# DillionLowry/NeuralCodecs

Measured on AMD Instinct MI355X. Metric: audio-seconds/sec encode+decode (x real-time), DAC-44.1kHz B=32, higher is better.
Workload: dtype f32; 1 GPU; DAC 44.1kHz 8kbps encode+decode, batch=32 x 1 s clips per GPU (BASELINE configs[1]); clips_per_gpu=32, global_batch=32, collective=none

## Files before the change

include/nc_mi355x.h:

```cpp
#ifndef NC_MI355X_H
#define NC_MI355X_H

#include <stddef.h>
#include <stdint.h>

#ifdef __cplusplus
extern "C" {
#endif

#define NC_API __attribute__((visibility("default")))

typedef enum {
    NC_OK = 0,
    NC_EINVAL = 1,
    NC_ENOTFOUND = 2,
    NC_ESTATE = 3,
    NC_EDEVICE = 4,
    NC_ENOMEM = 5,
    NC_EUNSUPPORTED = 6
} nc_status;

typedef struct nc_codec nc_codec;

NC_API const char* nc_last_error(void);
// ... 212 lines not shown
    NC_KC_COUNT = 13
} nc_kernel_class;

typedef struct {
    int64_t launches;
    double ms;
    double flops;
    double bytes;
} nc_profile_entry;

NC_API nc_status nc_codec_profile_enable(nc_codec* h, int32_t on);
NC_API nc_status nc_codec_profile_reset(nc_codec* h);
NC_API nc_status nc_codec_profile_read(nc_codec* h, nc_profile_entry* out);

typedef struct {
    int32_t B, Cin, Cout, K, stride, pad, dil, out_pad;
    int64_t Tin;
    int32_t transposed;
    int32_t tanh_out;
} nc_conv_desc;

NC_API nc_status nc_op_conv1d(int device_index, const nc_conv_desc* d, const float* x, const float* weight, const float* bias,
                              const float* alpha_in, const float* alpha_out, const float* residual, float* y, int64_t* Tout);
NC_API nc_status nc_op_conv1d_bench(int device_index, const nc_conv_desc* d, int32_t fuse, int32_t iters, double* avg_ms);
NC_API nc_status nc_op_res_unit(int device_index, int32_t B, int32_t C, int64_t T, int32_t dil, const float* x, const float* w7,
                                const float* b7, const float* a1, const float* a2, const float* w1, const float* b1,
                                int32_t fused, float* y, int32_t iters, double* avg_ms);
NC_API nc_status nc_op_vq_argmin(int device_index, const float* z_e, int32_t B, int32_t D, int64_t T, const float* codebook,
                                 int32_t N, int64_t* idx, float* st);
NC_API nc_status nc_op_euclid_rvq(int device_index, const float* residual, int32_t B, int32_t D, int64_t T, const float* codebooks,
                                  int32_t n_q, int32_t N, int32_t form, int64_t* codes, float* residual_out);
NC_API nc_status nc_op_fold_weight_norm(const float* v, const float* g, int64_t d0, int64_t inner, float* w);
NC_API nc_status nc_op_dwconv1d(int device_index, int32_t B, int32_t C, int64_t T, int32_t K, int32_t pad, int32_t dil, const float* x,
                                const float* w, const float* bias, const float* alpha_in, const float* alpha_out, float* y);
NC_API nc_status nc_op_layer_norm(int device_index, int32_t B, int32_t C, int64_t T, const float* x, const float* gamma,
                                  const float* beta, float* y);
NC_API nc_status nc_op_local_attn(int device_index, int32_t B, int32_t C, int64_t T, int32_t W, const float* qkv, const float* inv_freq,
                                  float* y);
NC_API nc_status nc_op_avg_pool(int device_index, int64_t rows, int64_t T, int32_t s, const float* x, float* y);
NC_API nc_status nc_op_snac_unit(int device_index, int32_t B, int32_t C, int64_t T, int32_t dil, const float* x, const float* w7,
                                 const float* b7, const float* a1, const float* a2, const float* w1, const float* b1,
                                 const float* alpha_next, int32_t fused, float* y);

#ifdef __cplusplus
}
#endif
// ... 2 lines not shown
```

neuralcodecs_amd/_lib.py:

```python
from __future__ import annotations

import ctypes as C
import os
import sys

_HERE = os.path.dirname(os.path.abspath(__file__))
LIB_PATH = os.path.join(_HERE, "libnc_mi355x.so")

NC_OK, NC_EINVAL, NC_ENOTFOUND, NC_ESTATE, NC_EDEVICE, NC_ENOMEM, NC_EUNSUPPORTED = range(7)
NC_KC_NAMES = ("conv_k7", "conv_k1", "conv_down", "conv_up", "conv_misc", "rvq", "elem", "dwconv", "norm", "attn", "lstm", "stem", "head")


class NcError(RuntimeError):
    """Base of engine errors (the reference's NeuralCodecException, Core/Exceptions/NeuralCodecException.cs:10-73)."""


class NcDeviceError(NcError):
    pass


class NcDacConfig(C.Structure):
    _fields_ = [("sample_rate", C.c_int32), ("encoder_dim", C.c_int32), ("n_encoder_rates", C.c_int32),
                ("encoder_rates", C.c_int32 * 8), ("decoder_dim", C.c_int32), ("n_decoder_rates", C.c_int32),
                ("decoder_rates", C.c_int32 * 8), ("latent_dim", C.c_int32), ("n_codebooks", C.c_int32),
# ... 108 lines not shown
    ("nc_audio_deinterleave_dev", C.c_int, [C.c_int, _P, C.c_int64, C.c_int32, _P, _P]),
    ("nc_audio_resample_linear_dev", C.c_int, [C.c_int, _P, C.c_int32, C.c_int64, C.c_int32, C.c_int32, _P, _P]),
    ("nc_group_unique_id", C.c_int, [_P]),
    ("nc_group_create_rank", C.c_int, [C.c_int32, C.c_int32, _P, _P, C.POINTER(_P)]),
    ("nc_group_create_local", C.c_int, [C.c_int32, C.POINTER(_P), C.POINTER(_P)]),
    ("nc_group_create_local_ex", C.c_int, [C.c_int32, C.POINTER(_P), C.c_uint32, C.POINTER(_P)]),
    ("nc_group_destroy", C.c_int, [_P]),
    ("nc_group_info", C.c_int, [_P, C.POINTER(C.c_int32), C.POINTER(C.c_int32)]),
    ("nc_group_set_code_bits", C.c_int, [_P, C.c_int32]),
    ("nc_group_dac_encode_allgather_dev", C.c_int, [_P, _P, C.c_int32, C.c_int64, C.c_int32, C.c_int32, _P, _P, _P]),
    ("nc_group_snac_encode_allgather_dev", C.c_int, [_P, _P, C.c_int32, C.c_int64, _P]),
    ("nc_group_wait", C.c_int, [_P]),
    ("nc_group_dac_encode_allgather", C.c_int, [_P, _P, C.c_int32, C.c_int64, C.c_int32, C.c_int32, _P, _P]),
    ("nc_group_snac_encode_allgather", C.c_int, [_P, _P, C.c_int32, C.c_int64, _P]),
    ("nc_group_dac_encode_allgather_local_dev", C.c_int, [_P, C.POINTER(_P), C.POINTER(C.c_int32), C.c_int64, C.c_int32, C.c_int32, C.POINTER(_P),
                                                          C.POINTER(_P), C.POINTER(_P)]),
    ("nc_group_snac_encode_allgather_local_dev", C.c_int, [_P, C.POINTER(_P), C.POINTER(C.c_int32), C.c_int64, C.POINTER(_P)]),
    ("nc_group_encodec_encode_allgather_dev", C.c_int, [_P, _P, C.c_int32, C.c_int64, _P, _P]),
    ("nc_group_encodec_encode_allgather_local_dev", C.c_int, [_P, C.POINTER(_P), C.POINTER(C.c_int32), C.c_int64, C.POINTER(_P), C.POINTER(_P)]),
    ("nc_codec_profile_enable", C.c_int, [_P, C.c_int32]),
    ("nc_codec_profile_reset", C.c_int, [_P]),
    ("nc_codec_profile_read", C.c_int, [_P, C.POINTER(NcProfileEntry)]),
    ("nc_op_conv1d", C.c_int, [C.c_int, C.POINTER(NcConvDesc), _P, _P, _P, _P, _P, _P, _P, C.POINTER(C.c_int64)]),
    ("nc_op_conv1d_bench", C.c_int, [C.c_int, C.POINTER(NcConvDesc), C.c_int32, C.c_int32, C.POINTER(C.c_double)]),
    ("nc_op_res_unit", C.c_int, [C.c_int, C.c_int32, C.c_int32, C.c_int64, C.c_int32, _P, _P, _P, _P, _P, _P, _P, C.c_int32, _P,
                                 C.c_int32, C.POINTER(C.c_double)]),
    ("nc_op_vq_argmin", C.c_int, [C.c_int, _P, C.c_int32, C.c_int32, C.c_int64, _P, C.c_int32, _P, _P]),
    ("nc_op_euclid_rvq", C.c_int, [C.c_int, _P, C.c_int32, C.c_int32, C.c_int64, _P, C.c_int32, C.c_int32, C.c_int32, _P, _P]),
    ("nc_op_fold_weight_norm", C.c_int, [_P, _P, C.c_int64, C.c_int64, _P]),
    ("nc_op_dwconv1d", C.c_int, [C.c_int, C.c_int32, C.c_int32, C.c_int64, C.c_int32, C.c_int32, C.c_int32, _P, _P, _P, _P, _P, _P]),
    ("nc_op_layer_norm", C.c_int, [C.c_int, C.c_int32, C.c_int32, C.c_int64, _P, _P, _P, _P]),
    ("nc_op_local_attn", C.c_int, [C.c_int, C.c_int32, C.c_int32, C.c_int64, C.c_int32, _P, _P, _P]),
    ("nc_op_avg_pool", C.c_int, [C.c_int, C.c_int64, C.c_int64, C.c_int32, _P, _P]),
    ("nc_op_snac_unit", C.c_int, [C.c_int, C.c_int32, C.c_int32, C.c_int64, C.c_int32, _P, _P, _P, _P, _P, _P, _P, _P, C.c_int32, _P]),
]


def lib():
    global _lib
    if _lib is not None:
        return _lib
    path = os.environ.get("NC_MI355X_LIB") or LIB_PATH
    if not os.path.exists(path):
        raise NcError(f"{path} is missing: build it with `python -c 'import __graft_entry__ as g; g.build()'` "
                      "(make -C neuralcodecs_amd/csrc). There is no fallback implementation.")
    if "torch" not in sys.modules:
# ... 73 lines not shown
```

neuralcodecs_amd/csrc/nc_api.hip:

```cpp
#include <algorithm>
#include <cmath>
#include <cstdio>
#include <fstream>

#include "nc_model.h"

using namespace nc;


namespace {

template <class F>
nc_status guard(F&& f) {
    try {
        f();
        return NC_OK;
    } catch (const Error& e) {
        set_last_error(e.what());
        return e.code;
    } catch (const std::bad_alloc&) {
        set_last_error("host allocation failed");
        return NC_ENOMEM;
    } catch (const std::exception& e) {
        set_last_error(e.what());
// ... 671 lines not shown
    return guard([&] {
        if (!d || !x || !weight || !y) fail(NC_EINVAL, "null argument");
        if (d->B <= 0 || d->Cin <= 0 || d->Cout <= 0 || d->K <= 0 || d->stride <= 0 || d->Tin <= 0) fail(NC_EINVAL, "bad conv shape");
        op_set_device(device_index);
        ConvLayer L;
        L.build(weight, bias, d->Cin, d->Cout, d->K, d->stride, d->pad, d->dil, d->out_pad, d->transposed != 0);
        const int64_t Tout = L.out_len(d->Tin);
        if (Tout <= 0) fail(NC_EINVAL, "empty output");
        if (Tout_p) *Tout_p = Tout;
        DevBuf dx, dy, dai, dao, dr;
        const size_t nx = (size_t)d->B * d->Cin * d->Tin * 4, ny = (size_t)d->B * d->Cout * Tout * 4;
        dx.reserve(nx); dy.reserve(ny);
        NC_HIP(hipMemcpy(dx.p, x, nx, hipMemcpyHostToDevice));
        NC_HIP(hipMemset(dy.p, 0, ny));
        if (alpha_in) { dai.reserve(d->Cin * 4); NC_HIP(hipMemcpy(dai.p, alpha_in, d->Cin * 4, hipMemcpyHostToDevice)); }
        if (alpha_out) { dao.reserve(d->Cout * 4); NC_HIP(hipMemcpy(dao.p, alpha_out, d->Cout * 4, hipMemcpyHostToDevice)); }
        if (residual) { dr.reserve(ny); NC_HIP(hipMemcpy(dr.p, residual, ny, hipMemcpyHostToDevice)); }
        ConvIO io{};
        io.x = dx.as<float>(); io.x_bstride = (int64_t)d->Cin * d->Tin; io.x_cstride = d->Tin; io.x_len = (int32_t)d->Tin; io.Tin = d->Tin;
        io.alpha_in = alpha_in ? dai.as<float>() : nullptr;
        io.alpha_out = alpha_out ? dao.as<float>() : nullptr;
        io.res = residual ? dr.as<float>() : nullptr;
        io.y = dy.as<float>(); io.y_bstride = (int64_t)d->Cout * Tout; io.y_cstride = Tout;
        io.epi = d->tanh_out ? EPI_TANH : 0;
        launch_conv(L, io, d->B, nullptr, nullptr);
        NC_HIP(hipDeviceSynchronize());
        NC_HIP(hipMemcpy(y, dy.p, ny, hipMemcpyDeviceToHost));
        dx.release(); dy.release(); dai.release(); dao.release(); dr.release(); L.release_all();
    });
}

nc_status nc_op_conv1d_bench(int device_index, const nc_conv_desc* d, int32_t fuse, int32_t iters, double* avg_ms) {
    return guard([&] {
        if (!d || !avg_ms || iters <= 0) fail(NC_EINVAL, "null argument");
        if (d->B <= 0 || d->Cin <= 0 || d->Cout <= 0 || d->K <= 0 || d->stride <= 0 || d->Tin <= 0) fail(NC_EINVAL, "bad conv shape");
        op_set_device(device_index);
        uint64_t st = 0x9E3779B97F4A7C15ull;
        auto rnd = [&]() {
            st = st * 6364136223846793005ull + 1442695040888963407ull;
            return (float)((int64_t)(st >> 40) - (1 << 23)) * (1.0f / (1 << 23));
        };
        const size_t nw = (size_t)d->Cin * d->Cout * d->K;
        std::vector<float> w(nw), bias(d->Cout), al(std::max(d->Cin, d->Cout));
        const float sc = 1.0f / std::sqrt((float)d->Cin * (d->transposed ? 2 : d->K));
        for (auto& v : w) v = rnd() * sc;
        for (auto& v : bias) v = rnd() * 0.1f;
// ... 260 lines not shown
```

neuralcodecs_amd/csrc/nc_chunk.hip:

```cpp
#include <algorithm>

#include "nc_limits.h"
#include "nc_model.h"

namespace nc {

namespace {

int64_t ceil_div(int64_t a, int64_t b) { return (a + b - 1) / b; }
int64_t round_up(int64_t a, int64_t m) { return ceil_div(a, m) * m; }

void halo_from_layers(const int32_t* er, int ne, const int32_t* dr, int nd, int final_reach, int W, int vq_max, int64_t align, nc_halo* out) {
    if (ne <= 0 || ne > 8 || nd <= 0 || nd > 8) fail(NC_EINVAL, "encoder/decoder rate lists must hold 1..8 entries");
    int64_t l = final_reach, r = final_reach, hop = 1;
    if (W > 1) { l += W - 1; r += W - 1; }
    for (int i = ne - 1; i >= 0; --i) {
        const int64_t s = er[i], p = (s + 1) / 2;
        if (s <= 0) fail(NC_EINVAL, "encoder rate must be positive");
        l = l * s + p; r = r * s + (2 * s - 1 - p);
        l += 39; r += 39;
        hop *= s;
    }
    l += 3; r += 3;
    int64_t a = 3, b = 3, H = 1;
    if (W > 1) { a += W - 1; b += W - 1; }
    for (int i = 0; i < nd; ++i) {
        const int64_t s = dr[i], p = (s + 1) / 2;
        if (s <= 0) fail(NC_EINVAL, "decoder rate must be positive");
        a = a * s + p; b = b * s + (2 * s - 1 - p);
        a += 39; b += 39;
        H *= s;
    }
    a += 3; b += 3;
    out->align = align;
    out->enc_left = round_up(ceil_div(r, hop) + (vq_max - 1), align);
    out->enc_right = round_up(ceil_div(l, hop) + (vq_max - 1), align);
    out->dec_left = round_up(ceil_div(a, H), align);
    out->dec_right = round_up(ceil_div(b, H), align);
}

int64_t pitch16(int64_t L) { return L >= 256 ? ((L + 15) & ~(int64_t)15) : L; }

int64_t auto_chunk(const nc_halo& h, bool decode) {
    const int64_t hmax = decode ? std::max(h.dec_left, h.dec_right) : std::max(h.enc_left, h.enc_right);
    return round_up(std::max<int64_t>(1024, 16 * hmax), h.align);
}

bool oneshot_fits(const int32_t* er, int ne, int enc_dim, const int32_t* dr, int nd, int dec_dim, ChunkKind kind, int64_t frames) {
    const int bm = 512;
    if (kind == CK_ENCODE) {
        int64_t L = frames;
        for (int i = 0; i < ne; ++i) L *= er[i];
        if (L > ((int64_t)1 << 30)) return false;
        return conv_rows_fit32(bm, pitch16(L), L);
    }
    if (kind == CK_DECODE) {
        int64_t L = frames;
        for (int i = 0; i < nd; ++i) {
            const int64_t s = dr[i], Lo = L * s, P = pitch16(Lo);
            const int Co = dec_dim >> (i + 1);
            if (!conv_rows_fit32(bm, P, Lo) || !conv_subpixel_fits32(Co, P, (int64_t)Co * P, Lo)) return false;
            L = Lo;
        }
        return true;
// ... 326 lines not shown
```

neuralcodecs_amd/csrc/nc_conv.hip:

```cpp
#include <algorithm>
#include <cstdlib>
#include <mutex>
#include <set>

#include "nc_conv.h"
#include "nc_limits.h"

namespace nc {

typedef void (*conv_kernel_fn)(const ConvArgs);
conv_kernel_fn conv_kernel_table_k1(int, int);
int conv_kernel_cb_k1();
int conv_kernel_nx_k1();
conv_kernel_fn conv_kernel_table_k2(int, int);
int conv_kernel_cb_k2();
int conv_kernel_nx_k2();
conv_kernel_fn conv_kernel_table_k3(int, int);
int conv_kernel_cb_k3();
int conv_kernel_nx_k3();
conv_kernel_fn conv_kernel_table_k4(int, int);
int conv_kernel_cb_k4();
int conv_kernel_nx_k4();
conv_kernel_fn conv_kernel_table_k6(int, int);
int conv_kernel_cb_k6();
int conv_kernel_nx_k6();
conv_kernel_fn conv_kernel_table_k7(int, int);
int conv_kernel_cb_k7();
int conv_kernel_nx_k7();
conv_kernel_fn conv_kernel_table_k8(int, int);
int conv_kernel_cb_k8();
int conv_kernel_nx_k8();
conv_kernel_fn conv_kernel_table_k10(int, int);
int conv_kernel_cb_k10();
int conv_kernel_nx_k10();
conv_kernel_fn conv_kernel_table_k16(int, int);
int conv_kernel_cb_k16();
int conv_kernel_nx_k16();

#define NC_K_CASES(X) X(1) X(2) X(3) X(4) X(6) X(7) X(8) X(10) X(16)

conv_kernel_fn conv_kernel_table_fused_k7(int, int);
conv_kernel_fn conv_kernel_table_xv_k7(int);
conv_kernel_fn conv_kernel_table_xv_fused_k7(int);
conv_kernel_fn conv_kernel_table_xv_sub_k2(int);
conv_kernel_fn conv_kernel_table_xv_subg_k2(int);
conv_kernel_fn conv_kernel_table_sub_k2(int, int);
conv_kernel_fn conv_kernel_table_subg_k2(int, int);
conv_kernel_fn conv_kernel_table_dist_k16(int, int);
conv_kernel_fn conv_kernel_table_dist_sub_k2(int, int);
conv_kernel_fn conv_kernel_table_sub_narrow_k2(int);
conv_kernel_fn conv_kernel_table_fusedw_k7(int, int);
conv_kernel_fn conv_kernel_table_slim_k3(int, int);
conv_kernel_fn conv_kernel_table_slim_k7(int, int);
conv_kernel_fn conv_kernel_table_narrow_k2(int);
conv_kernel_fn conv_kernel_table_narrow_k3(int);
conv_kernel_fn conv_kernel_table_narrow_k7(int);
conv_kernel_fn conv_kernel_table_narrow_k16(int);
static conv_kernel_fn narrow_kernel(int K, int TM) {
    switch (K) {
        case 2: return conv_kernel_table_narrow_k2(TM);
        case 3: return conv_kernel_table_narrow_k3(TM);
        case 7: return conv_kernel_table_narrow_k7(TM);
        case 16: return conv_kernel_table_narrow_k16(TM);
    }
    return nullptr;
}
conv_kernel_fn conv_kernel_table_in2_k4(int, int);
conv_kernel_fn conv_kernel_table_in2_k8(int, int);
// ... 602 lines not shown
        if (io.epi & EPI_NOISE) fail(NC_ESTATE, "internal: noise epilogue on the multiply-shift sub-pixel form");
        a.sub_stride = L.sub_stride; a.sub_cout = L.Cout; a.sub_magic = magic_div(L.sub_stride, L.rows() + 256);
        if (!conv_subpixel_fits32(L.Cout, io.y_cstride, io.y_bstride, Tout))
            fail(NC_EUNSUPPORTED, "conv output of %lld samples per row exceeds the 32-bit offsets of the sub-pixel form", (long long)io.y_cstride);
    }
    a.Tout = (int32_t)Tout;
    if (!conv_rows_fit32(c.BM(), io.y_cstride, Tout))
        fail(NC_EUNSUPPORTED, "conv output rows of %lld samples exceed the 32-bit tile offsets", (long long)io.y_cstride);
    int sx;
    if (L.transposed) {
        sx = 1; a.stride = 1; a.dil = -1; a.pad = 0;
        a.n_cols = (int32_t)(io.Tin + L.Ktaps - 1);
        a.y_tstride = L.stride; a.y_toff = -L.pad;
        a.n_phase = L.n_phase;
    } else {
        sx = L.stride; a.stride = L.stride; a.dil = L.dil; a.pad = L.pad;
        a.n_cols = (int32_t)Tout;
        a.y_tstride = 1; a.y_toff = 0;
        a.n_phase = 1;
    }
    const int ad = a.dil < 0 ? -a.dil : a.dil;
    a.xneg = a.dil < 0 ? (L.Ktaps - 1) * ad : 0;
    int xv_extra = 0;
    conv_kernel_fn xv_fn = nullptr;
    {
        static const bool no_xv = env_flag("NC_NO_XV");
        static const bool no_xr = env_flag("NC_NO_XR");
        static const bool no_xv_k7 = env_flag("NC_NO_XV_K7");
        static const int64_t xv_k7_min = env_int("NC_XV_K7_MIN_COLS", 0);
        const bool xv_k7 = !no_xv_k7 && n_cols_all >= xv_k7_min;
        const bool two_tap = L.sub_stride && L.n_phase == 1 && c.K == 2 && c.CB == 16 && !io.alpha_in && !io.fuse_k1;
        const bool k7 = xv_k7 && !L.transposed && !L.sub_stride && c.K == 7 && c.CB == 8 && L.stride == 1 && !fused_wide;
        const int vw = two_tap ? 4 : 2;
        if (!no_xv && !no_xr && (two_tap || k7) && c.TN == 2 && c.NW == 4 && c.TM >= 2 && c.TM <= 4 && !narrow && !flat && !dist_small_fn &&
            !slim && !in_mode && !io.x2 && !io.gn_part && sx == 1 && L.Cin % c.CB == 0 && io.x_len % vw == 0 &&
            io.x_cstride % 16 == 0 && io.x_bstride % 16 == 0 && (reinterpret_cast<uintptr_t>(io.x) & 63) == 0) {
            xv_extra = (vw - (a.pad + a.xneg) % vw) % vw;
            if ((BN - 1) * sx + (L.Ktaps - 1) * ad + 1 + xv_extra <= 320) {
                xv_fn = two_tap ? (L.sub_shift ? conv_kernel_table_xv_sub_k2(c.TM) : conv_kernel_table_xv_subg_k2(c.TM))
                                : (io.fuse_k1 ? conv_kernel_table_xv_fused_k7(c.TM) : conv_kernel_table_xv_k7(c.TM));
            }
            if (xv_fn) { a.xneg += xv_extra; a.epi |= EPI_XVEC; }
            else xv_extra = 0;
        }
    }
    a.xw = (BN - 1 + (flat ? (flat_S - 1) * flat_hc : 0)) * sx + (L.Ktaps - 1) * ad + 1 + xv_extra;
    a.nchunk = (a.xw + 63) / 64;
    a.xwp = (a.nchunk * 64 + sx - 1) / sx;
    a.xrow = sx == 1 ? a.nchunk * 64 : sx * a.xwp;
    a.n_co_tiles = (L.rows() + BM - 1) / BM;
    a.n_t_tiles = (a.n_cols + BN - 1) / BN;
    {
        static const bool no_xr = env_flag("NC_NO_XR");
        if (no_xr) a.epi |= EPI_NO_XR;
    }
    a.Bc = B; a.flat = 0; a.flat_px = a.flat_pc = 0x1fffffff; a.flat_hc = 0;
    if (flat) {
        a.flat = 1; a.flat_pc = (int32_t)flat_pitch; a.flat_hc = flat_hc; a.flat_px = (int32_t)(flat_pitch + flat_hc) * sx;
        a.n_t_tiles = (int32_t)(((int64_t)B * flat_pitch + BN - 1) / BN);
        a.B = 1;
    }
    a.n_cb = (L.Cin + CB - 1) / CB;
    a.co_group = 1;
    a.n_items = CB * a.nchunk;
    if (a.n_items > NW * nx)
        fail(NC_EUNSUPPORTED, "conv K=%d stride=%d dil=%d: input window of %d words per channel exceeds the staging registers",
// ... 67 lines not shown
        }
    }
#endif
    hipLaunchKernelGGL(fn, dim3((unsigned)grid), dim3(64 * c.NW), lds, stream, a);
    NC_HIP(hipGetLastError());
    if (prof && prof->on) prof->end(stream);
#ifdef NC_CONV_TRACE
    if (trace_now) {
        std::vector<unsigned long long> hb((size_t)16 * 8 * 8 * 8);
        NC_HIP(hipStreamSynchronize(stream));
        NC_HIP(hipMemcpy(hb.data(), trace_buf.p, hb.size() * 8, hipMemcpyDeviceToHost));
        if (FILE* f = std::fopen(trace_file, "wb")) {
            const int hdr[8] = {16, c.NW, 8, 8, c.TM, c.TN, c.K, (a.epi & EPI_XVEC) ? 1 : 0};
            std::fwrite(hdr, sizeof(int), 8, f);
            std::fwrite(hb.data(), 8, hb.size(), f);
            std::fclose(f);
        }
        trace_buf.release();
    }
#endif
    {
        FILE* lf = launch_log();
        if (lf) {
            std::fprintf(lf, "conv_mfma %d %lld %d %d %d %lld %d\n", L.kclass, (long long)grid * 64 * c.NW, L.Cin, L.Cout, L.K,
                         (long long)io.Tin, io.fuse_k1 ? 1 : 0);
            std::fflush(lf);
        }
    }
}

}
```

neuralcodecs_amd/csrc/nc_conv_kernel.hip.h:

```cpp
#pragma once
#include <hip/hip_runtime.h>

#include "nc_conv.h"
#include "nc_math.h"
#include "nc_frag.h"
#include "nc_gn.h"

#include <type_traits>
#include <utility>

#ifdef NC_CONV_TRACE
#define NC_TRACE_WGS 16
#ifndef NC_TRACE_WG0
#define NC_TRACE_WG0 1024
#endif
#define NC_TRACE_CB0 8
#define NC_TRACE_NCB 8
#endif

namespace nc {

typedef float f32x16 __attribute__((ext_vector_type(16)));
typedef float f32x4 __attribute__((ext_vector_type(4)));

struct nc_rt_flag {
    bool v;
    __device__ constexpr operator bool() const { return v; }
};
typedef __attribute__((address_space(1))) const void* nc_gptr;
typedef __attribute__((address_space(3))) void* nc_lptr;

template <int TM, int TN, int K, int CB, int NX, bool FUSE = false, int OCC = 2, int NW = 4, bool DIST = false, int SUB = 0,
          bool IN2 = false, bool XVK = false>
__global__ __launch_bounds__(64 * NW, OCC) void conv_mfma_kernel(const ConvArgs p) {
    constexpr int NT = 64 * NW;
    constexpr int BM = 32 * TM;
    constexpr int BNW = 32 * TN;
    constexpr int BN = NW * BNW;
    constexpr int KB = CB * K;
    constexpr int KP = KB / 2;
    constexpr int A_FLOATS = KB * BM;
    constexpr int A_VEC = A_FLOATS / 4;
    constexpr int NA = (A_VEC + NT - 1) / NT;
// ... 19 lines not shown
    unsigned long long* const trace_p = (!IN2 && p.x2 != nullptr && blockIdx.x >= NC_TRACE_WG0 && blockIdx.x < NC_TRACE_WG0 + NC_TRACE_WGS)
        ? reinterpret_cast<unsigned long long*>(const_cast<float*>(p.x2)) + ((size_t)(blockIdx.x - NC_TRACE_WG0) * 8 + (tid >> 6)) * NC_TRACE_NCB * 8 : nullptr;
#define NC_STAMP(cb, slot)                                                                                         \
    do {                                                                                                            \
        if (trace_p && (cb) >= NC_TRACE_CB0 && (cb) < NC_TRACE_CB0 + NC_TRACE_NCB && (tid & 63) == 0)               \
            trace_p[((cb) - NC_TRACE_CB0) * 8 + (slot)] = __builtin_amdgcn_s_memtime();                             \
    } while (0)
#else
#define NC_STAMP(cb, slot) do {} while (0)
#endif
    const int swave = wave;
    const int stid = tid;

    const int nwg = gridDim.x;
    const int bid = blockIdx.x;
    int lin = nc_xcd_tile_id(bid, nwg);
    const int phase = __builtin_amdgcn_readfirstlane(lin % p.n_phase);
    lin /= p.n_phase;
    const int co_in = __builtin_amdgcn_readfirstlane(lin % p.co_group);
    lin /= p.co_group;
    const int t_tile = __builtin_amdgcn_readfirstlane(lin % p.n_t_tiles);
    lin /= p.n_t_tiles;
    const int co_tile = __builtin_amdgcn_readfirstlane((lin / p.B) * p.co_group + co_in);
    const bool flatm = XVK ? false : (p.flat != 0);
    const int b = __builtin_amdgcn_readfirstlane(flatm ? (t_tile * BN) / p.flat_pc : lin % p.B);
    const int col0 = flatm ? t_tile * BN - b * p.flat_pc : t_tile * BN;
    const int flat_px = XVK ? 0x1fffffff : p.flat_px, flat_pc = XVK ? 0x1fffffff : p.flat_pc;
    const int flat_hc = XVK ? 0 : p.flat_hc;
    auto seg_of = [&](int r, int pitch) __attribute__((always_inline)) -> int { return (int)(r >= pitch) + (int)(r >= 2 * pitch) + (int)(r >= 3 * pitch); };

    const int s = p.stride;
    const int xs0 = col0 * s - p.pad - p.xneg;

    const f32x4* const wbase =
        reinterpret_cast<const f32x4*>(p.w + (int64_t)phase * p.w_phase_stride + (int64_t)co_tile * p.n_cb * A_FLOATS);
    const float* const xb = p.x + (int64_t)b * p.x_bstride;
    const float* const xb2 = IN2 ? p.x2 + (int64_t)b * p.x_bstride : nullptr;

    float* const As0 = smem;
    float* const Xs0 = smem + 2 * A_FLOATS;

    const int nchunk = p.nchunk, chunk_magic = p.chunk_magic, stride_magic = p.stride_magic;
    const int xwp = p.xwp, xrow = p.xrow, xbuf = p.xbuf, Cin = p.Cin, x_len = p.x_len, n_cb = p.n_cb;
    const unsigned x_cstride = (unsigned)p.x_cstride;
    const float* const alpha_in = p.alpha_in;
    const int in_mode = XVK ? 0 : p.in_mode;
    const float in_mu = (in_mode & 1) ? p.in_stats[2 * b] : 0.0f, in_rs = (in_mode & 1) ? p.in_stats[2 * b + 1] : 1.0f;
    const float in_mu2 = (IN2 && (in_mode & 1)) ? p.in_stats2[2 * b] : 0.0f, in_rs2 = (IN2 && (in_mode & 1)) ? p.in_stats2[2 * b + 1] : 1.0f;
    int tap[K];
#pragma unroll
    for (int k = 0; k < K; ++k) tap[k] = p.tapoff[k];
// ... 16 lines not shown
        const int gp = xs0 + jw - sg * flat_px;
        xg[i] = (unsigned)min(sg, p.Bc - 1 - b) * (unsigned)p.x_bstride + (unsigned)min(max(gp, 0), x_len - 1);
        if ((b + sg < p.Bc) & (gp >= 0) & (gp < x_len)) okm |= 1u << i;
        if (in_mode & 4) {
            int q = gp - p.in_left;
            q = q < 0 ? -q : q;
            if (q >= p.in_Lz) q = 2 * (p.in_Lz - 1) - q;
            if (!((q >= 0) & (q < p.in_L))) okm &= ~(1u << i);
            xg[i] = (unsigned)min(sg, p.Bc - 1 - b) * (unsigned)p.x_bstride + (unsigned)min(max(q, 0), p.in_L - 1);
        }
    }
    const bool tile_allok = __builtin_amdgcn_ballot_w64(okm != (NX >= 32 ? ~0u : (1u << NX) - 1u)) == 0;
    constexpr bool XVCAND = XVK;
    static_assert(!XVK || (TN == 2 && NW == 4 && !IN2 && !DIST && ((K == 2 && SUB != 0 && !FUSE) || (K == 7 && SUB == 0))),
                  "XV-only instances: two-tap sub-pixel or k = 7, 256-column tiles");
    constexpr int XVW = K == 2 ? 4 : 2;
    constexpr int XVROW = 320;
    constexpr int XVN = CB * XVROW / XVW;
    constexpr int NV = XVCAND ? (XVN + NT - 1) / NT : 1;
    typedef float xv_t __attribute__((ext_vector_type(XVW)));
    constexpr bool use_xv = XVCAND;
    unsigned xvo[NV];
    unsigned xvok = 0;
    int xvc[(XVCAND && K == 7) ? NV : 1];
    xv_t rxv[NV];
    f32x4 rav[XVCAND ? NA : 1];
    if constexpr (XVCAND) {
        {
#pragma unroll
            for (int n = 0; n < NV; ++n) {
                const int f = min(tid + NT * n, XVN - 1);
                const int ch = f / (XVROW / XVW), q = f - ch * (XVROW / XVW);
                const int gp = xs0 + XVW * q;
                const bool ok = (gp >= 0) & (gp + XVW - 1 < x_len);
                xvo[n] = (unsigned)ch * x_cstride + (unsigned)(ok ? gp : 0);
                if constexpr (K == 7) xvc[n] = ch;
                if (ok) xvok |= 1u << n;
            }
        }
    }
    const bool xv_allok = __builtin_amdgcn_ballot_w64(xvok != (1u << NV) - 1u) == 0;
    auto xv_issue = [&](int cbn) __attribute__((always_inline)) {
        if constexpr (XVCAND) {
            const float* base = xb + (size_t)((unsigned)(cbn * CB) * x_cstride);
#pragma unroll
            for (int n = 0; n < NV; ++n) rxv[n] = *reinterpret_cast<const xv_t*>(base + xvo[n]);
            const f32x4* src = wbase + (size_t)cbn * A_VEC;
#pragma unroll
            for (int n = 0; n < NA; ++n) rav[n] = (src + NT * n)[(A_VEC % NT == 0) ? (unsigned)stid : min((unsigned)stid, (unsigned)(A_VEC - 1 - NT * n))];
        }
    };
    auto xv_store = [&](int cbn, float* Ad, float* Xd, auto allok_tag, auto snake_tag) __attribute__((always_inline)) {
        if constexpr (XVCAND) {
#pragma unroll
            for (int n = 0; n < NA; ++n)
                if ((A_VEC % NT == 0) || stid + NT * n < A_VEC) reinterpret_cast<f32x4*>(Ad)[stid + NT * n] = rav[n];
            if constexpr (K == 7 && decltype(snake_tag)::value) {
                nc_f2 xv[NV], a[NV], iv[NV];
#pragma unroll
                for (int n = 0; n < NV; ++n) {
                    const float2 al = Al[cbn * CB + xvc[n]];
                    a[n] = nc_f2{al.x, al.x}; iv[n] = nc_f2{al.y, al.y};
                    xv[n] = nc_f2{rxv[n][0], rxv[n][1]};
                    if constexpr (!decltype(allok_tag)::value)
                        if (!((xvok >> n) & 1u)) xv[n] = nc_f2{0.0f, 0.0f};
                }
                nc_snakef2_m_rows<NV>(xv, a, iv);
#pragma unroll
                for (int n = 0; n < NV; ++n)
                    if ((XVN % NT == 0) || tid + NT * n < XVN) reinterpret_cast<xv_t*>(Xd)[tid + NT * n] = xv_t{xv[n][0], xv[n][1]};
            } else {
#pragma unroll
                for (int n = 0; n < NV; ++n) {
                    xv_t v = rxv[n];
                    if constexpr (!decltype(allok_tag)::value)
                        if (!((xvok >> n) & 1u)) v = xv_t(0.0f);
                    if ((XVN % NT == 0) || tid + NT * n < XVN) reinterpret_cast<xv_t*>(Xd)[tid + NT * n] = v;
                }
            }
        }
    };
    auto xv_stage = [&](int cb, float* An, float* Xn) __attribute__((always_inline)) {
        if constexpr (XVCAND) {
            if (K == 7 && alpha_in != nullptr) {
                if (xv_allok) xv_store(cb + 1, An, Xn, std::true_type{}, std::true_type{});
                else xv_store(cb + 1, An, Xn, std::false_type{}, std::true_type{});
            } else {
                if (xv_allok) xv_store(cb + 1, An, Xn, std::true_type{}, std::false_type{});
                else xv_store(cb + 1, An, Xn, std::false_type{}, std::false_type{});
            }
            if (cb + 2 < n_cb) xv_issue(cb + 2);
        }
    };
    auto issue_group_to = [&](int cbn, auto gtag, f32x4 (&ra)[GA], float (&rx)[GXX]) __attribute__((always_inline)) {
        constexpr int g = decltype(gtag)::value;
        const f32x4* src = wbase + (size_t)cbn * A_VEC;
        nc_static_for<GX>([&](auto ut) __attribute__((always_inline)) {
            constexpr int u = decltype(ut)::value, i = g * GX + u;
            if constexpr (i < NX) {
// ... 959 lines not shown
```

neuralcodecs_amd/csrc/nc_dac.hip:

```cpp
#include <cstdlib>
#include <cstring>

#include "nc_model.h"

namespace nc {

Codec::~Codec() {
    if (own_stream) (void)hipStreamDestroy(own_stream);
}

void Codec::init_device(int device_index) {
    int n = 0;
    if (hipGetDeviceCount(&n) != hipSuccess || n <= 0) fail(NC_EDEVICE, "no HIP device available (the engine has no CPU fallback)");
    if (device_index < 0 || device_index >= n) fail(NC_EINVAL, "device index %d out of range (0..%d)", device_index, n - 1);
    device = device_index;
    NC_HIP(hipSetDevice(device));
    hipDeviceProp_t prop;
    NC_HIP(hipGetDeviceProperties(&prop, device));
    if (std::strncmp(prop.gcnArchName, "gfx950", 6) != 0)
        fail(NC_EDEVICE, "device %d is %s; this engine is built for gfx950 (MI355X) only", device, prop.gcnArchName);
    cu_count = prop.multiProcessorCount;
    lds_per_cu = prop.maxSharedMemoryPerMultiProcessor;
    NC_HIP(hipStreamCreateWithFlags(&own_stream, hipStreamNonBlocking));
    stream = own_stream;
// ... 158 lines not shown
            load_alpha(b, q + ".block.2.alpha", out_dim, dec[bi].ru[u].a2);
            load_wn_conv(b, q + ".block.3", dec[bi].ru[u].c1, out_dim, out_dim, 1, 1, 0, 1, false, NC_KC_CONV_K1);
        }
    }
    snprintf(nm, sizeof nm, "decoder.model.%d.alpha", cfg.n_decoder_rates + 1);
    load_alpha(b, nm, out_dim, dec_alpha_out);
    snprintf(nm, sizeof nm, "decoder.model.%d", cfg.n_decoder_rates + 2);
    load_wn_conv(b, nm, dec_out, out_dim, 1, 7, 1, 3, 1, false, NC_KC_HEAD);
    NC_HIP(hipDeviceSynchronize());
    loaded = true;
}

int64_t DacModel::decoded_len(int64_t fr) const {
    int64_t L = fr;
    for (int i = 0; i < cfg.n_decoder_rates; ++i) {
        const int s = cfg.decoder_rates[i];
        L = (L - 1) * s - 2 * ((s + 1) / 2) + 2 * s;
    }
    return L;
}

static int64_t row_pitch(int64_t L) {
    static const bool on = env_flag("NC_DAC_PITCH");
    return (on && L >= 256) ? ((L + 15) & ~(int64_t)15) : L;
}

float* DacModel::run_res_unit(ResUnit& ru, int dil, float* cur, int C, int64_t L, int B, int& cur_idx, const float* alpha_next) {
    (void)dil;
    const int64_t P = row_pitch(L);
    const int h_idx = (cur_idx + 1) % 3, o_idx = (cur_idx + 2) % 3;
    float* h = act[h_idx].as<float>();
    float* o = act[o_idx].as<float>();
    ConvIO io{};
    io.x = cur; io.x_bstride = (int64_t)C * P; io.x_cstride = P; io.x_len = (int32_t)L; io.Tin = L;
    io.alpha_in = ru.a1.as<float>(); io.alpha_out = ru.a2.as<float>();
    static const bool wide_192 = env_flag("NC_WIDE_FUSE_192");
    if (fuse_res_units && can_fuse_res_unit(ru.c7, ru.c1) && (C != 192 || wide_192)) {
        io.res = cur; io.fuse_k1 = &ru.c1; io.alpha_out2 = alpha_next;
        io.y = o; io.y_bstride = (int64_t)C * P; io.y_cstride = P;
        launch_conv(ru.c7, io, B, stream, &prof);
        cur_idx = o_idx;
        return o;
    }
    io.y = h; io.y_bstride = (int64_t)C * P; io.y_cstride = P;
    launch_conv(ru.c7, io, B, stream, &prof);
    ConvIO i2{};
    i2.x = h; i2.x_bstride = (int64_t)C * P; i2.x_cstride = P; i2.x_len = (int32_t)L; i2.Tin = L;
// ... 188 lines not shown
```

neuralcodecs_amd/csrc/nc_util.hip:

```cpp
#include <cmath>
#include <mutex>
#include <set>
#include <tuple>

#include "nc_common.h"
#include "nc_model.h"

namespace nc {

static thread_local std::string g_last_error;
void set_last_error(const char* msg) { g_last_error = msg ? msg : ""; }
const char* get_last_error() { return g_last_error.c_str(); }

namespace {
struct EnvRow { const char* name; char kind; const char* doc; };
const EnvRow kEnv[] = {
    {"NC_NO_FLAT", 'b', "one-clip column tiles instead of the flattened (clip, column) axis"},
    {"NC_NO_FLAT_GN", 'b', "one-clip tiles wherever GroupNorm sums are emitted"},
    {"NC_CO_GROUP", 'i', "cap of the row-tile groups (1 = one weight panel per XCD)"},
    {"NC_NO_WIDE_FUSE", 'b', "no whole-channel fused residual units (C = 256)"},
    {"NC_WIDE_FUSE_192", 'b', "whole-channel fused unit at C = 192 as well"},
    {"NC_NO_FUSE", 'b', "every residual unit in two launches"},
    {"NC_NO_TILE_ALTS", 'b', "primary row-tile height only"},
    {"NC_TM_PICK", 'i', "force a packed row-tile variant"},
// ... 12 lines not shown
    {"NC_NO_SKINNY", 'b', "no skinny projection kernel (Cout <= 16)"},
    {"NC_NO_THIN", 'b', "PCM heads through the matrix-core template"},
    {"NC_THIN_NO_VEC", 'p', "scalar window loads in the thin-output kernel"},
    {"NC_NO_THIN_INM", 'b', "summed copy + plain head instead of the input-mode head"},
    {"NC_NO_STEM", 'b', "stems through the matrix-core template"},
    {"NC_NO_TINY_TILES", 'b', "no smallest-tile rule for tiny grids"},
    {"NC_TINY_BLOCKS", 'i', "grid size below which the tiny-grid rule applies (256)"},
    {"NC_NO_DIST_SMALL", 'b', "segmented staging on small grids"},
    {"NC_DIST_MAX_GRID", 'i', "largest grid that takes distributed staging (768)"},
    {"NC_NO_CONV_SMALL", 'b', "no short-row 16x16x4 kernel"},
    {"NC_SMALL_MAX_GRID", 'i', "largest short-row grid (2048)"},
    {"NC_SMALL_WIDE_BELOW", 'i', "template grid below which the 32-column short-row form is taken (512)"},
    {"NC_SMALL_K1_COLS", 'i', "columns up to which k = 1 layers take the short-row kernel (4096; 0 = off)"},
    {"NC_SMALL_TN", 'i', "force the short-row column tiles (1 | 2 | 4)"},
    {"NC_SMALL_ROLLED", 'b', "rolled short-row loop"},
    {"NC_DAC_RVQ_STAGEWISE", 'p', "DAC quantizer stage by stage"},
    {"NC_EUCLID_NO_MFMA", 'p', "vector Euclidean codebook search"},
    {"NC_ENCODEC_NO_FUSE", 'b', "padded / activated copies instead of the fused SConv1d input mode"},
    {"NC_ENCODEC_NO_OVERLAP", 'b', "segment groups one after the other"},
    {"NC_NO_GN_FUSE", 'b', "stand-alone GroupNorm sums"},
    {"NC_NO_GN_FINISH", 'b', "separate GroupNorm final launch"},
    {"NC_NO_IN2", 'b', "summed copies instead of the two-input staging mode"},
    {"NC_NO_CONV3S", 'b', "windowed k = 3 instead of the streaming kernel"},
    {"NC_DAC_PITCH", 'b', "DAC activation rows at pitch L rounded up to 16 samples (64-byte aligned rows: the 696-step layers take the XV-only instances; measured slower)"},
    {"NC_NO_DOWN2", 'b', "Encodec 48 kHz encoder: the windowed two-input instance for the stride-2 down-convolution instead of the streaming kernel"},
    {"NC_NO_DOWN4", 'b', "Encodec 48 kHz encoder: summed copy + windowed instance for the stride-4 down-convolution instead of the streaming kernel"},
    {"NC_NO_DOWN5", 'b', "Encodec 48 kHz encoder: summed copy + windowed instance for the stride-5 down-convolution instead of the streaming kernel"},
    {"NC_NO_UP_PITCH", 'b', "Encodec transposed convolutions write dense rows (the trimmed view of the stride-5 layer then starts on an odd sample)"},
    {"NC_NO_UP4", 'b', "Encodec 48 kHz decoder: summed copy + windowed instance for the stride-4 up-convolution instead of the streaming kernel"},
    {"NC_NO_UP2", 'b', "Encodec 48 kHz decoder: the windowed two-input instance for the stride-2 up-convolution instead of the streaming kernel"},
    {"NC_RMS_TWO_PASS", 'b', "Encodec RMS scale as two launches (chunk sums, final) instead of the one-launch form"},
    {"NC_NO_RES_A", 'b', "residual blocks of the Encodec 48 kHz outer stages: shortcut and k = 3 branch as two launches instead of the fused first pass"},
    {"NC_SYNC_ACQUIRE", 'b', "agent-scope acquire fence behind the persistent LSTM's flag poll and in front of the in-launch GroupNorm finish"},
    {"NC_LSTM_STEPWISE", 'b', "one LSTM launch per step"},
    {"NC_LSTM_CHUNKS", 'i', "layer-pipeline chunks of the per-layer persistent LSTM (6; 1 = layers in sequence)"},
    {"NC_LSTM_EVEN_CHUNKS", 'b', "equal LSTM chunks"},
    {"NC_LSTM_UB", 'i', "hidden-unit blocks per LSTM workgroup (2 | 4)"},
    {"NC_LSTM_NO_HTILE", 'b', "persistent LSTM: every wavefront fetches its own h operands, W_hh in LDS (the form before the LDS h tile)"},
    {"NC_LSTM_NO_ELU", 'b', "the consumer applies the ELU behind an SLSTM"},
    {"NC_LSTM_FAKE_TIMEOUT", 'b', "tests: report the first persistent LSTM launch as timed out"},
    {"NC_SNAC_NO_FUSE", 'b', "SNAC residual units in two launches (depthwise, pointwise)"},
    {"NC_SNAC_FUSE_MIN_COLS", 'i', "columns (clips x steps) from which the one-launch SNAC residual unit is taken (65536)"},
    {"NC_SNAC_FUSE_MAX_ELEMS", 'i', "channels x steps of ONE clip up to which the one-launch SNAC residual unit is taken (2^30: its 32-bit lane offsets; tests lower it)"},
    {"NC_SNAC_UNIT_TRACE", 's', "file for the in-kernel stamps of the first one-launch SNAC residual unit at C = 96"},
    {"NC_DW_NO_VEC", 'b', "scalar depthwise kernel"},
    {"NC_LN_TILE", 'i', "LayerNorm tile width (8 | 16; 0 = one thread per column)"},
// ... 191 lines not shown
```

neuralcodecs_amd/ops.py:

```python
from __future__ import annotations

import ctypes as C

import numpy as np

from . import _lib


def _p(a):
    return None if a is None else a.ctypes.data


def conv1d(x, weight, bias=None, stride=1, pad=0, dil=1, alpha_in=None, alpha_out=None, residual=None, transposed=False,
           out_pad=0, tanh_out=False, device_index=0):
    x = np.ascontiguousarray(x, np.float32); w = np.ascontiguousarray(weight, np.float32)
    B, Cin, Tin = x.shape
    if transposed:
        Cout, K = w.shape[1], w.shape[2]
        Tout = (Tin - 1) * stride - 2 * pad + K + out_pad
    else:
        Cout, K = w.shape[0], w.shape[2]
        Tout = (Tin + 2 * pad - dil * (K - 1) - 1) // stride + 1
    d = _lib.NcConvDesc(B, Cin, Cout, K, stride, pad, dil, out_pad, Tin, 1 if transposed else 0, 1 if tanh_out else 0)
    f = lambda a: None if a is None else np.ascontiguousarray(a, np.float32)
    b, ai, ao, r = f(bias), f(alpha_in), f(alpha_out), f(residual)
    y = np.empty((B, Cout, Tout), np.float32)
    to = C.c_int64()
    _lib.check(_lib.lib().nc_op_conv1d(device_index, C.byref(d), x.ctypes.data, w.ctypes.data, _p(b), _p(ai), _p(ao), _p(r),
                                       y.ctypes.data, C.byref(to)))
    assert to.value == Tout
    return y


def res_unit(x, w7, b7, a1, a2, w1, b1, dil=1, fused=True, iters=0, device_index=0):
    f = lambda a: np.ascontiguousarray(a, np.float32)
    x, w7, b7, a1, a2, w1, b1 = map(f, (x, w7, b7, a1, a2, w1, b1))
    B, Cc, T = x.shape
    y = np.empty_like(x)
    ms = C.c_double()
    _lib.check(_lib.lib().nc_op_res_unit(device_index, B, Cc, T, dil, x.ctypes.data, w7.ctypes.data, b7.ctypes.data, a1.ctypes.data,
                                         a2.ctypes.data, w1.ctypes.data, b1.ctypes.data, 1 if fused else 0, y.ctypes.data, iters,
                                         C.byref(ms)))
    return (y, ms.value) if iters > 0 else y


def vq_argmin(z_e, codebook, device_index=0):
    z = np.ascontiguousarray(z_e, np.float32); cb = np.ascontiguousarray(codebook, np.float32)
    B, D, T = z.shape
    idx = np.empty((B, T), np.int64); st = np.empty_like(z)
    _lib.check(_lib.lib().nc_op_vq_argmin(device_index, z.ctypes.data, B, D, T, cb.ctypes.data, cb.shape[0], idx.ctypes.data,
                                          st.ctypes.data))
    return idx, st
# ... 68 lines not shown
```

Before: 594.5 audio-seconds/sec.

## Add XV-vectorized flat-column conv instances and pad short DAC rows to 16

Adds new conv kernel instantiations that combine vectorized (XV) input staging with the flattened batch-column layout. They handle segment boundaries across batch rows with per-vector partial-validity masks. DAC activation rows of 32 to 1024 samples now use a pitch rounded up to 16, so those layers satisfy the alignment needed for the vector path. The aim is faster input staging for the short-row deep layers, at the cost of padded memory, extra masking logic, and the risk of wrong edge handling. A pitched conv test entry point is also added.

Result: no change. 595.0 audio-seconds/sec, median of 3 (+0.1%).

```diff
diff --git a/include/nc_mi355x.h b/include/nc_mi355x.h
--- a/include/nc_mi355x.h
+++ b/include/nc_mi355x.h
@@ -258,6 +258,9 @@
 
 NC_API nc_status nc_op_conv1d(int device_index, const nc_conv_desc* d, const float* x, const float* weight, const float* bias,
                               const float* alpha_in, const float* alpha_out, const float* residual, float* y, int64_t* Tout);
+NC_API nc_status nc_op_conv1d_pitched(int device_index, const nc_conv_desc* d, int64_t x_pitch, int64_t y_pitch, const float* x,
+                                      const float* weight, const float* bias, const float* alpha_in, const float* alpha_out,
+                                      const float* residual, float* y, int64_t* Tout);
 NC_API nc_status nc_op_conv1d_bench(int device_index, const nc_conv_desc* d, int32_t fuse, int32_t iters, double* avg_ms);
 NC_API nc_status nc_op_res_unit(int device_index, int32_t B, int32_t C, int64_t T, int32_t dil, const float* x, const float* w7,
                                 const float* b7, const float* a1, const float* a2, const float* w1, const float* b1,
diff --git a/neuralcodecs_amd/_lib.py b/neuralcodecs_amd/_lib.py
--- a/neuralcodecs_amd/_lib.py
+++ b/neuralcodecs_amd/_lib.py
@@ -154,6 +154,7 @@
     ("nc_codec_profile_reset", C.c_int, [_P]),
     ("nc_codec_profile_read", C.c_int, [_P, C.POINTER(NcProfileEntry)]),
     ("nc_op_conv1d", C.c_int, [C.c_int, C.POINTER(NcConvDesc), _P, _P, _P, _P, _P, _P, _P, C.POINTER(C.c_int64)]),
+    ("nc_op_conv1d_pitched", C.c_int, [C.c_int, C.POINTER(NcConvDesc), C.c_int64, C.c_int64, _P, _P, _P, _P, _P, _P, _P, C.POINTER(C.c_int64)]),
     ("nc_op_conv1d_bench", C.c_int, [C.c_int, C.POINTER(NcConvDesc), C.c_int32, C.c_int32, C.POINTER(C.c_double)]),
     ("nc_op_res_unit", C.c_int, [C.c_int, C.c_int32, C.c_int32, C.c_int64, C.c_int32, _P, _P, _P, _P, _P, _P, _P, C.c_int32, _P,
                                  C.c_int32, C.POINTER(C.c_double)]),
diff --git a/neuralcodecs_amd/csrc/nc_api.hip b/neuralcodecs_amd/csrc/nc_api.hip
--- a/neuralcodecs_amd/csrc/nc_api.hip
+++ b/neuralcodecs_amd/csrc/nc_api.hip
@@ -717,6 +717,40 @@
         io.alpha_out = alpha_out ? dao.as<float>() : nullptr;
         io.res = residual ? dr.as<float>() : nullptr;
         io.y = dy.as<float>(); io.y_bstride = (int64_t)d->Cout * Tout; io.y_cstride = Tout;
+        io.epi = d->tanh_out ? EPI_TANH : 0;
+        launch_conv(L, io, d->B, nullptr, nullptr);
+        NC_HIP(hipDeviceSynchronize());
+        NC_HIP(hipMemcpy(y, dy.p, ny, hipMemcpyDeviceToHost));
+        dx.release(); dy.release(); dai.release(); dao.release(); dr.release(); L.release_all();
+    });
+}
+
+nc_status nc_op_conv1d_pitched(int device_index, const nc_conv_desc* d, int64_t x_pitch, int64_t y_pitch, const float* x, const float* weight,
+                               const float* bias, const float* alpha_in, const float* alpha_out, const float* residual, float* y, int64_t* Tout_p) {
+    return guard([&] {
+        if (!d || !x || !weight || !y) fail(NC_EINVAL, "null argument");
+        if (d->B <= 0 || d->Cin <= 0 || d->Cout <= 0 || d->K <= 0 || d->stride <= 0 || d->Tin <= 0) fail(NC_EINVAL, "bad conv shape");
+        op_set_device(device_index);
+        ConvLayer L;
+        L.build(weight, bias, d->Cin, d->Cout, d->K, d->stride, d->pad, d->dil, d->out_pad, d->transposed != 0);
+        const int64_t Tout = L.out_len(d->Tin);
+        if (Tout <= 0) fail(NC_EINVAL, "empty output");
+        if (x_pitch < d->Tin || y_pitch < Tout) fail(NC_EINVAL, "row pitch below the row length");
+        if (Tout_p) *Tout_p = Tout;
+        DevBuf dx, dy, dai, dao, dr;
+        const size_t nx = (size_t)d->B * d->Cin * x_pitch * 4, ny = (size_t)d->B * d->Cout * y_pitch * 4;
+        dx.reserve(nx); dy.reserve(ny);
+        NC_HIP(hipMemcpy(dx.p, x, nx, hipMemcpyHostToDevice));
+        NC_HIP(hipMemcpy(dy.p, y, ny, hipMemcpyHostToDevice));
+        if (alpha_in) { dai.reserve(d->Cin * 4); NC_HIP(hipMemcpy(dai.p, alpha_in, d->Cin * 4, hipMemcpyHostToDevice)); }
+        if (alpha_out) { dao.reserve(d->Cout * 4); NC_HIP(hipMemcpy(dao.p, alpha_out, d->Cout * 4, hipMemcpyHostToDevice)); }
+        if (residual) { dr.reserve(ny); NC_HIP(hipMemcpy(dr.p, residual, ny, hipMemcpyHostToDevice)); }
+        ConvIO io{};
+        io.x = dx.as<float>(); io.x_bstride = (int64_t)d->Cin * x_pitch; io.x_cstride = x_pitch; io.x_len = (int32_t)d->Tin; io.Tin = d->Tin;
+        io.alpha_in = alpha_in ? dai.as<float>() : nullptr;
+        io.alpha_out = alpha_out ? dao.as<float>() : nullptr;
+        io.res = residual ? dr.as<float>() : nullptr;
+        io.y = dy.as<float>(); io.y_bstride = (int64_t)d->Cout * y_pitch; io.y_cstride = y_pitch;
         io.epi = d->tanh_out ? EPI_TANH : 0;
         launch_conv(L, io, d->B, nullptr, nullptr);
         NC_HIP(hipDeviceSynchronize());
diff --git a/neuralcodecs_amd/csrc/nc_chunk.hip b/neuralcodecs_amd/csrc/nc_chunk.hip
--- a/neuralcodecs_amd/csrc/nc_chunk.hip
+++ b/neuralcodecs_amd/csrc/nc_chunk.hip
@@ -39,7 +39,7 @@
     out->dec_right = round_up(ceil_div(b, H), align);
 }
 
-int64_t pitch16(int64_t L) { return L >= 256 ? ((L + 15) & ~(int64_t)15) : L; }
+int64_t pitch16(int64_t L) { return L >= 32 ? ((L + 15) & ~(int64_t)15) : L; }
 
 int64_t auto_chunk(const nc_halo& h, bool decode) {
     const int64_t hmax = decode ? std::max(h.dec_left, h.dec_right) : std::max(h.enc_left, h.enc_right);
diff --git a/neuralcodecs_amd/csrc/nc_conv.hip b/neuralcodecs_amd/csrc/nc_conv.hip
--- a/neuralcodecs_amd/csrc/nc_conv.hip
+++ b/neuralcodecs_amd/csrc/nc_conv.hip
@@ -44,6 +44,8 @@
 conv_kernel_fn conv_kernel_table_xv_fused_k7(int);
 conv_kernel_fn conv_kernel_table_xv_sub_k2(int);
 conv_kernel_fn conv_kernel_table_xv_subg_k2(int);
+conv_kernel_fn conv_kernel_table_xvf_k7(int);
+conv_kernel_fn conv_kernel_table_xvf_sub_k2(int);
 conv_kernel_fn conv_kernel_table_sub_k2(int, int);
 conv_kernel_fn conv_kernel_table_subg_k2(int, int);
 conv_kernel_fn conv_kernel_table_dist_k16(int, int);
@@ -692,6 +694,7 @@
     const int ad = a.dil < 0 ? -a.dil : a.dil;
     a.xneg = a.dil < 0 ? (L.Ktaps - 1) * ad : 0;
     int xv_extra = 0;
+    bool xv_flat = false;
     conv_kernel_fn xv_fn = nullptr;
     {
         static const bool no_xv = env_flag("NC_NO_XV");
@@ -712,6 +715,22 @@
             }
             if (xv_fn) { a.xneg += xv_extra; a.epi |= EPI_XVEC; }
             else xv_extra = 0;
+        }
+        static const bool no_xv_flat = env_flag("NC_NO_XV_FLAT");
+        if (!no_xv && !no_xr && !no_xv_flat && flat && (two_tap ? L.sub_shift != 0 : k7) && !io.fuse_k1 && c.TN == 2 && c.NW == 4 && !narrow &&
+            !dist_small_fn && !slim && !in_mode && !io.x2 && !io.gn_part && sx == 1 && L.Cin % c.CB == 0 &&
+            io.x_cstride % 16 == 0 && io.x_bstride % 16 == 0 && (reinterpret_cast<uintptr_t>(io.x) & 63) == 0 &&
+            (int64_t)c.CB * io.x_cstride + 3 * io.x_bstride + io.x_len < ((int64_t)1 << 32)) {
+            const int extra = (vw - (a.pad + a.xneg) % vw) % vw;
+            const int64_t pc = (flat_pitch + vw - 1) / vw * vw;
+            const int hc = ((L.Ktaps - 1) * ad + extra + vw - 1) / vw * vw;
+            const int S = (int)((BN - 2) / pc) + 2;
+            conv_kernel_fn f = two_tap ? conv_kernel_table_xvf_sub_k2(c.TM) : conv_kernel_table_xvf_k7(c.TM);
+            if (f && S <= 4 && (BN - 1 + (S - 1) * hc) + (L.Ktaps - 1) * ad + 1 + extra <= 320) {
+                xv_fn = f; xv_extra = extra; xv_flat = true;
+                flat_pitch = pc; flat_hc = hc; flat_S = S;
+                a.xneg += xv_extra; a.epi |= EPI_XVEC;
+            }
         }
     }
     a.xw = (BN - 1 + (flat ? (flat_S - 1) * flat_hc : 0)) * sx + (L.Ktaps - 1) * ad + 1 + xv_extra;
@@ -825,8 +844,8 @@
     {
         FILE* lf = launch_log();
         if (lf) {
-            std::fprintf(lf, "conv_mfma %d %lld %d %d %d %lld %d\n", L.kclass, (long long)grid * 64 * c.NW, L.Cin, L.Cout, L.K,
-                         (long long)io.Tin, io.fuse_k1 ? 1 : 0);
+            std::fprintf(lf, "conv_mfma %d %lld %d %d %d %lld %d %s %d %d\n", L.kclass, (long long)grid * 64 * c.NW, L.Cin, L.Cout, L.K,
+                         (long long)io.Tin, io.fuse_k1 ? 1 : 0, xv_flat ? "xvf" : xv_fn ? "xv" : "legacy", a.flat, (int)(a.B * a.n_t_tiles));
             std::fflush(lf);
         }
     }
diff --git a/neuralcodecs_amd/csrc/nc_conv_kernel.hip.h b/neuralcodecs_amd/csrc/nc_conv_kernel.hip.h
--- a/neuralcodecs_amd/csrc/nc_conv_kernel.hip.h
+++ b/neuralcodecs_amd/csrc/nc_conv_kernel.hip.h
@@ -18,7 +18,18 @@
 #define NC_TRACE_NCB 8
 #endif
 
+#ifdef NC_CONV_XVF
+#define conv_mfma_kernel conv_mfma_kernel_xvf
+#define get_conv_kernel get_conv_xvf_kernel
+#endif
+
 namespace nc {
+
+#ifdef NC_CONV_XVF
+constexpr bool kXvFlat = true;
+#else
+constexpr bool kXvFlat = false;
+#endif
 
 typedef float f32x16 __attribute__((ext_vector_type(16)));
 typedef float f32x4 __attribute__((ext_vector_type(4)));
@@ -84,11 +95,12 @@
     const int t_tile = __builtin_amdgcn_readfirstlane(lin % p.n_t_tiles);
     lin /= p.n_t_tiles;
     const int co_tile = __builtin_amdgcn_readfirstlane((lin / p.B) * p.co_group + co_in);
-    const bool flatm = XVK ? false : (p.flat != 0);
+    constexpr bool XVF = XVK && kXvFlat;
+    const bool flatm = XVF ? true : XVK ? false : (p.flat != 0);
     const int b = __builtin_amdgcn_readfirstlane(flatm ? (t_tile * BN) / p.flat_pc : lin % p.B);
     const int col0 = flatm ? t_tile * BN - b * p.flat_pc : t_tile * BN;
-    const int flat_px = XVK ? 0x1fffffff : p.flat_px, flat_pc = XVK ? 0x1fffffff : p.flat_pc;
-    const int flat_hc = XVK ? 0 : p.flat_hc;
+    const int flat_px = (XVK && !XVF) ? 0x1fffffff : p.flat_px, flat_pc = (XVK && !XVF) ? 0x1fffffff : p.flat_pc;
+    const int flat_hc = (XVK && !XVF) ? 0 : p.flat_hc;
     auto seg_of = [&](int r, int pitch) __attribute__((always_inline)) -> int { return (int)(r >= pitch) + (int)(r >= 2 * pitch) + (int)(r >= 3 * pitch); };
 
     const int s = p.stride;
@@ -151,6 +163,7 @@
     constexpr bool use_xv = XVCAND;
     unsigned xvo[NV];
     unsigned xvok = 0;
+    unsigned xvpc = 0;
     int xvc[(XVCAND && K == 7) ? NV : 1];
     xv_t rxv[NV];
     f32x4 rav[XVCAND ? NA : 1];
@@ -160,11 +173,22 @@
             for (int n = 0; n < NV; ++n) {
                 const int f = min(tid + NT * n, XVN - 1);
                 const int ch = f / (XVROW / XVW), q = f - ch * (XVROW / XVW);
+                if constexpr (XVF) {
+                    const int sg = seg_of(col0 + XVW * q, flat_px);
+                    const int gp = xs0 + XVW * q - sg * flat_px;
+                    const bool any = (b + sg < p.Bc) & (gp >= 0) & (gp < x_len);
+                    const bool ok = any & (gp + XVW - 1 < x_len);
+                    xvo[n] = (unsigned)ch * x_cstride + (unsigned)min(sg, p.Bc - 1 - b) * (unsigned)p.x_bstride + (unsigned)(any ? gp : 0);
+                    if constexpr (K == 7) xvc[n] = ch;
+                    if (ok) xvok |= 1u << n;
+                    else if (any) xvpc |= (unsigned)(x_len - gp) << (2 * n);
+                } else {
                 const int gp = xs0 + XVW * q;
                 const bool ok = (gp >= 0) & (gp + XVW - 1 < x_len);
                 xvo[n] = (unsigned)ch * x_cstride + (unsigned)(ok ? gp : 0);
                 if constexpr (K == 7) xvc[n] = ch;
                 if (ok) xvok |= 1u << n;
+                }
             }
         }
     }
@@ -191,8 +215,12 @@
                     const float2 al = Al[cbn * CB + xvc[n]];
                     a[n] = nc_f2{al.x, al.x}; iv[n] = nc_f2{al.y, al.y};
                     xv[n] = nc_f2{rxv[n][0], rxv[n][1]};
-                    if constexpr (!decltype(allok_tag)::value)
+                    if constexpr (!decltype(allok_tag)::value) {
+                        if constexpr (XVF) {
+                            if (!((xvok >> n) & 1u)) xv[n] = nc_f2{((xvpc >> (2 * n)) & 3u) ? xv[n][0] : 0.0f, 0.0f};
+                        } else
                         if (!((xvok >> n) & 1u)) xv[n] = nc_f2{0.0f, 0.0f};
+                    }
                 }
                 nc_snakef2_m_rows<NV>(xv, a, iv);
 #pragma unroll
@@ -202,8 +230,16 @@
 #pragma unroll
                 for (int n = 0; n < NV; ++n) {
                     xv_t v = rxv[n];
-                    if constexpr (!decltype(allok_tag)::value)
+                    if constexpr (!decltype(allok_tag)::value) {
+                        if constexpr (XVF) {
+                            if (!((xvok >> n) & 1u)) {
+                                const unsigned cnt = (xvpc >> (2 * n)) & 3u;
+#pragma unroll
+                                for (int e = 0; e < XVW; ++e) v[e] = (unsigned)e < cnt ? v[e] : 0.0f;
+                            }
+                        } else
                         if (!((xvok >> n) & 1u)) v = xv_t(0.0f);
+                    }
                     if ((XVN % NT == 0) || tid + NT * n < XVN) reinterpret_cast<xv_t*>(Xd)[tid + NT * n] = v;
                 }
             }
diff --git a/neuralcodecs_amd/csrc/nc_conv_xvf2.hip b/neuralcodecs_amd/csrc/nc_conv_xvf2.hip
--- /dev/null
+++ b/neuralcodecs_amd/csrc/nc_conv_xvf2.hip
@@ -0,0 +1,10 @@
+#define NC_CONV_XVF 1
+#include "nc_conv_kernel.hip.h"
+namespace nc {
+conv_kernel_fn conv_kernel_table_xvf_sub_k2(int TM) {
+    switch (TM) {
+        case 3: return get_conv_kernel<3, 2, 2, 16, 20, false, 2, 4, false, 1, false, true>();
+    }
+    return nullptr;
+}
+}
diff --git a/neuralcodecs_amd/csrc/nc_conv_xvf7.hip b/neuralcodecs_amd/csrc/nc_conv_xvf7.hip
--- /dev/null
+++ b/neuralcodecs_amd/csrc/nc_conv_xvf7.hip
@@ -0,0 +1,11 @@
+#define NC_CONV_XVF 1
+#include "nc_conv_kernel.hip.h"
+namespace nc {
+conv_kernel_fn conv_kernel_table_xvf_k7(int TM) {
+    switch (TM) {
+        case 2: return get_conv_kernel<2, 2, 7, 8, 10, false, 2, 4, false, 0, false, true>();
+        case 3: return get_conv_kernel<3, 2, 7, 8, 10, false, 2, 4, false, 0, false, true>();
+    }
+    return nullptr;
+}
+}
diff --git a/neuralcodecs_amd/csrc/nc_dac.hip b/neuralcodecs_amd/csrc/nc_dac.hip
--- a/neuralcodecs_amd/csrc/nc_dac.hip
+++ b/neuralcodecs_amd/csrc/nc_dac.hip
@@ -204,7 +204,9 @@
 
 static int64_t row_pitch(int64_t L) {
     static const bool on = env_flag("NC_DAC_PITCH");
-    return (on && L >= 256) ? ((L + 15) & ~(int64_t)15) : L;
+    static const bool no_xv_flat = env_flag("NC_NO_XV_FLAT");
+    const bool short_rows = !no_xv_flat && L >= 32 && L <= 1024;
+    return ((on && L >= 256) || short_rows) ? ((L + 15) & ~(int64_t)15) : L;
 }
 
 float* DacModel::run_res_unit(ResUnit& ru, int dil, float* cur, int C, int64_t L, int B, int& cur_idx, const float* alpha_next) {
diff --git a/neuralcodecs_amd/csrc/nc_util.hip b/neuralcodecs_amd/csrc/nc_util.hip
--- a/neuralcodecs_amd/csrc/nc_util.hip
+++ b/neuralcodecs_amd/csrc/nc_util.hip
@@ -58,6 +58,7 @@
     {"NC_NO_GN_FINISH", 'b', "separate GroupNorm final launch"},
     {"NC_NO_IN2", 'b', "summed copies instead of the two-input staging mode"},
     {"NC_NO_CONV3S", 'b', "windowed k = 3 instead of the streaming kernel"},
+    {"NC_NO_XV_FLAT", 'b', "legacy conv instances on the flattened column axis and dense DAC rows of 32 .. 1024 samples (no XV-only flat instances, no 16-sample row pitch)"},
     {"NC_DAC_PITCH", 'b', "DAC activation rows at pitch L rounded up to 16 samples (64-byte aligned rows: the 696-step layers take the XV-only instances; measured slower)"},
     {"NC_NO_DOWN2", 'b', "Encodec 48 kHz encoder: the windowed two-input instance for the stride-2 down-convolution instead of the streaming kernel"},
     {"NC_NO_DOWN4", 'b', "Encodec 48 kHz encoder: summed copy + windowed instance for the stride-4 down-convolution instead of the streaming kernel"},
diff --git a/neuralcodecs_amd/ops.py b/neuralcodecs_amd/ops.py
--- a/neuralcodecs_amd/ops.py
+++ b/neuralcodecs_amd/ops.py
@@ -28,6 +28,27 @@
     to = C.c_int64()
     _lib.check(_lib.lib().nc_op_conv1d(device_index, C.byref(d), x.ctypes.data, w.ctypes.data, _p(b), _p(ai), _p(ao), _p(r),
                                        y.ctypes.data, C.byref(to)))
+    assert to.value == Tout
+    return y
+
+
+def conv1d_pitched(x, t_in, weight, y_pitch, bias=None, stride=1, pad=0, dil=1, alpha_in=None, alpha_out=None, transposed=False,
+                   y_fill=0.0, device_index=0):
+    x = np.ascontiguousarray(x, np.float32); w = np.ascontiguousarray(weight, np.float32)
+    B, Cin, x_pitch = x.shape
+    if transposed:
+        Cout, K = w.shape[1], w.shape[2]
+        Tout = (t_in - 1) * stride - 2 * pad + K
+    else:
+        Cout, K = w.shape[0], w.shape[2]
+        Tout = (t_in + 2 * pad - dil * (K - 1) - 1) // stride + 1
+    d = _lib.NcConvDesc(B, Cin, Cout, K, stride, pad, dil, 0, t_in, 1 if transposed else 0, 0)
+    f = lambda a: None if a is None else np.ascontiguousarray(a, np.float32)
+    b, ai, ao = f(bias), f(alpha_in), f(alpha_out)
+    y = np.full((B, Cout, y_pitch), y_fill, np.float32)
+    to = C.c_int64()
+    _lib.check(_lib.lib().nc_op_conv1d_pitched(device_index, C.byref(d), x_pitch, y_pitch, x.ctypes.data, w.ctypes.data, _p(b), _p(ai),
+                                               _p(ao), None, y.ctypes.data, C.byref(to)))
     assert to.value == Tout
     return y
 
```
